# typesense/typesense

Hardware: AMD Instinct MI355X
Metric: queries/sec, 10M-doc keyword 3-term AND top-100 (Topster 250) (higher is better)
Workload: dtype u32/i64

## Files before the change

### typesense_amd/csrc/kw_find2.hip.h

```cpp
#pragma once

#ifndef TSGPU_F2_SPAN
#define TSGPU_F2_SPAN 12
#endif
#ifndef TSGPU_F2_FAST
#define TSGPU_F2_FAST 1
#endif
static const int KW_F2_SPAN = TSGPU_F2_SPAN;
#ifndef TSGPU_F2_WAVES
#define TSGPU_F2_WAVES 7
#endif
#ifdef TSGPU_HIP_EMU
#define KW_F2_WAVES
#else
#define KW_F2_WAVES __attribute__((amdgpu_waves_per_eu(TSGPU_F2_WAVES)))
#endif
#ifndef TSGPU_F2_QUAD
#define TSGPU_F2_QUAD 0
#endif
static const bool KW_F2_QUAD = TSGPU_F2_QUAD != 0;
static const bool KW_F2_FAST = TSGPU_F2_FAST != 0;
#ifndef TSGPU_F2_MIDSLABS
#define TSGPU_F2_MIDSLABS 0
#endif
// ... 6 lines not shown
#else
#define KW_F2_LOOP_BARRIER() __syncthreads()
#endif


template <int TMAX, bool COUNT = false>
__device__ __forceinline__ void kw_find2_body(const IndexView& ix, const KwQueryDev* __restrict__ queries, const KwWorkItem* __restrict__ work, const KwPartials& part,
                                              uint32_t* __restrict__ hits_all, const uint64_t* __restrict__ hit_off, const uint32_t bid) {
    __shared__ KwSmem<TMAX, 512, false, true, true> sm;
    __shared__ uint32_t wave_cnt_b[2][KW_THREADS / 64];
    uint32_t* __restrict__ hits = hits_all + hit_off[bid] * (uint64_t)(TMAX + 1);
    __shared__ KwQueryDev sq;
    const uint32_t t = threadIdx.x;
    const KwWorkItem wi = work[bid];
    uint32_t cb_ids = 0, cb_meta = 0, cb_tile = 0, cb_probe = 0, cb_rec = 0;
    {
        const uint32_t* src = (const uint32_t*)(queries + wi.query);
        uint32_t* dst = (uint32_t*)&sq;
        for (uint32_t i = t; i < sizeof(KwQueryDev) / 4; i += KW_THREADS) { dst[i] = src[i]; if constexpr (COUNT) cb_meta += 4; }
    }
    if (t == 0) { sm.q1_cnt = 0; sm.qf_cnt = 0; sm.tk_cnt = 0; sm.have_thr = 0; sm.n_match = 0; sm.n_emit = 0; sm.off_words = 0; }
    __syncthreads();
    const KwQueryDev& q = sq;
    const uint32_t T = q.n_lists;
    const ListDesc dA = ix.lists[q.list[q.probe_order[0]]];
    const ListDesc dB = ix.lists[q.list[q.probe_order[T >= 2 ? 1 : 0]]];
    const uint32_t* __restrict__ blB = ix.blk_last + dB.blk_base;
    const BlockIds* __restrict__ biA = ix.blk_ids + dA.blk_base;
    const BlockIds* __restrict__ biB = ix.blk_ids + dB.blk_base;
    const uint32_t* __restrict__ idwA = ix.ids_payload + dA.ids_base;
    const uint32_t* __restrict__ idwB = ix.ids_payload + dB.ids_base;
    const uint32_t lane = t & 63, wave = t >> 6;
    const BlockIds PAD = {0xFFFFFFFFu, 0xFFFFFFFFu, 0u, 0u};
    if constexpr (COUNT) { if (lane == 0) cb_meta += 2 * (uint32_t)sizeof(ListDesc) + 16; }

    auto load_id_raw = [&](const BlockIds& m, uint32_t slot) -> uint32_t {
        const uint32_t n = m.n_ids_bits & 0xFFFF;
        const uint32_t s2 = slot < n ? slot : 0;
        const uint32_t* __restrict__ w = idwA + m.ids_woff;
        if constexpr (COUNT) { if (slot < n) cb_ids += (m.n_ids_bits >> 16) == 16 ? 2u : 4u; }
        return (m.n_ids_bits >> 16) == 16 ? (uint32_t)((const uint16_t*)w)[s2] : w[s2];
    };
    const uint32_t nB = T >= 2 ? dB.n_blocks : 0u;
    auto load_window = [&](uint32_t base) -> BlockIds {
        if constexpr (COUNT) { if (base + lane < nB) cb_meta += 16; }
        return base + lane < nB ? biB[base + lane] : PAD;
    };
    uint32_t abase = wi.blk_begin;
    auto load_awin = [&](uint32_t base) -> BlockIds { const uint32_t bb = base + lane; if constexpr (COUNT) { if (bb < wi.blk_end) cb_meta += 16; } return biA[bb < wi.blk_end ? bb : wi.blk_end - 1]; };
    BlockIds awin = load_awin(abase);
    auto meta = [&](uint32_t bb) -> BlockIds {
        const int j = (int)((bb < wi.blk_end ? bb : wi.blk_end - 1) - abase);
        BlockIds m;
        m.first_id = (uint32_t)__builtin_amdgcn_readlane((int)awin.first_id, j);
        m.last_id = (uint32_t)__builtin_amdgcn_readlane((int)awin.last_id, j);
        m.ids_woff = (uint32_t)__builtin_amdgcn_readlane((int)awin.ids_woff, j);
        m.n_ids_bits = (uint32_t)__builtin_amdgcn_readlane((int)awin.n_ids_bits, j);
        return m;
    };

    uint32_t wbase = 0, wver = 0;
    BlockIds win = load_window(0), nxt = load_window(32);
    uint32_t win_dirty = 1;
    struct Plan { uint32_t mode, rlo, rhi, w_begin, W, ver, base, buf; };
    constexpr int PIPE_WORDS = KW_FIND_PIPE_WORDS;
    constexpr int TILE_WORDS = KW_FIND_TILE_WORDS;
    static_assert(TILE_WORDS == 2 * PIPE_WORDS * KW_THREADS, "two tile buffers: one searched, one being filled");
    constexpr int HALF = PIPE_WORDS * KW_THREADS;
    uint32_t tbuf = 0;
    auto make_plan = [&](uint32_t lo_id, uint32_t hi_id) -> Plan {
        Plan P; P.mode = 4; P.rlo = P.rhi = P.w_begin = P.W = 0; P.ver = wver; P.base = wbase; P.buf = 0;
        if (T < 2) return P;
        unsigned long long mk = __ballot(win.last_id >= lo_id ? 1 : 0);
        if (mk != 0 && (uint32_t)__builtin_ctzll(mk) >= 32) {
            wbase += 32; win = nxt; nxt = load_window(wbase + 32); win_dirty = 1;
            mk = __ballot(win.last_id >= lo_id ? 1 : 0);
        }
        if (mk == 0) {
            uint32_t lo = wbase + 64, hi = dB.n_blocks;
            while (lo < hi) { const uint32_t mid = (lo + hi) >> 1; if constexpr (COUNT) { if (lane == 0) cb_meta += 4; } if (blB[mid] >= lo_id) hi = mid; else lo = mid + 1; }
            wbase = lo; win = load_window(wbase); nxt = load_window(wbase + 32); win_dirty = 1;
            mk = __ballot(win.last_id >= lo_id ? 1 : 0);
        }
        P.rlo = (uint32_t)__builtin_ctzll(mk);
        P.base = wbase;
        if (wbase + P.rlo >= dB.n_blocks) { P.mode = 3; return P; }
        const unsigned long long mh = __ballot(win.last_id >= hi_id ? 1 : 0);
// ... 5 lines not shown
            if (t < 64) { sm.bw_last[wver][t] = win.last_id; sm.bw_first[wver][t] = win.first_id; sm.bw_woff[wver][t] = win.ids_woff; sm.bw_nb[wver][t] = win.n_ids_bits; }
            win_dirty = 0;
        }
        P.ver = wver;
        uint32_t has_breaks = dB.flags & LIST_HAS_BREAKS;
        KW_UNIFORM_OPAQUE(has_breaks);
        if (has_breaks) {
            const uint32_t w_endw = win.ids_woff + packed_words(win.n_ids_bits & 0xFFFF, win.n_ids_bits >> 16);
            const uint32_t nxt_woff = (uint32_t)__shfl(win.ids_woff, (int)((lane + 1) & 63));
            const bool brk = lane >= P.rlo && lane < P.rhi && w_endw != nxt_woff;
            if (__ballot(brk ? 1 : 0) != 0) { P.mode = 2; return P; }
        }
        P.w_begin = (uint32_t)__builtin_amdgcn_readlane((int)win.ids_woff, (int)P.rlo);
        const uint32_t nb_hi = (uint32_t)__builtin_amdgcn_readlane((int)win.n_ids_bits, (int)P.rhi);
        P.W = (uint32_t)__builtin_amdgcn_readlane((int)win.ids_woff, (int)P.rhi) + packed_words(nb_hi & 0xFFFF, nb_hi >> 16) - P.w_begin;
        if (P.W <= (uint32_t)(PIPE_WORDS * KW_THREADS)) {
            P.mode = 0;
            tbuf ^= 1; P.buf = tbuf;
            const uint32_t* lane_src = idwB + P.w_begin + t;
            uint32_t* lds_wave_base = sm.btile + tbuf * HALF + wave * 64;
#if TSGPU_F2_MIDSLABS
            if (P.W <= 2u * KW_THREADS) kw_glds_slabs<2>(lane_src, lds_wave_base);
            else if (PIPE_WORDS > 4 && P.W <= 4u * KW_THREADS) kw_glds_slabs<4>(lane_src, lds_wave_base);
            else kw_glds_slabs<PIPE_WORDS>(lane_src, lds_wave_base);
            if constexpr (COUNT) cb_tile += 4u * (P.W <= 2u * KW_THREADS ? 2u : ((PIPE_WORDS > 4 && P.W <= 4u * KW_THREADS) ? 4u : (uint32_t)PIPE_WORDS));
#else
            if (P.W <= 2u * KW_THREADS) kw_glds_slabs<2>(lane_src, lds_wave_base);
            else kw_glds_slabs<PIPE_WORDS>(lane_src, lds_wave_base);
            if constexpr (COUNT) cb_tile += 4u * (P.W <= 2u * KW_THREADS ? 2u : (uint32_t)PIPE_WORDS);
#endif
        } else P.mode = KW_F2_ROUNDS ? 1 : 2;
        return P;
    };

    uint32_t a_first, a_nb, b_first, b_nb;
    uint32_t araw0, araw1;
    Plan P;
    {
        const BlockIds mA = meta(wi.blk_begin), mB = meta(wi.blk_begin + 1);
        araw0 = load_id_raw(mA, t); araw1 = load_id_raw(mB, t);
        P = make_plan(mA.first_id, wi.blk_begin + 1 < wi.blk_end ? mB.last_id : mA.last_id);
        a_first = mA.first_id; a_nb = mA.n_ids_bits; b_first = mB.first_id; b_nb = mB.n_ids_bits;
    }
    const uint32_t has_deadline = q.deadline_rem_us;
    uint32_t q1n = 0, qfn = 0, par = 0, qh = 0;
    KW_PROF_DECL
// ... 33 lines not shown
    auto drain_q1 = [&]() { while (q1n >= (uint32_t)KW_THREADS) probe_batch(KW_THREADS); };

    for (uint32_t b = wi.blk_begin, it = 0; b < wi.blk_end; b += 2, it++) {
        if (P.mode == 3) break;
        uint32_t Tl = T;
        KW_UNIFORM_OPAQUE(Tl);
        KW_PROF(8)
        kw_glds_wait();
        KW_PROF(1)
        if (has_deadline) { if ((it & 7) == 0 && kw_out_of_time<true>(KW_RELOAD_VIEW(ix), q, wi.query, &sm.stop)) break; }
        const bool two = b + 1 < wi.blk_end;
        const uint32_t n0 = a_nb & 0xFFFF, n1 = two ? (b_nb & 0xFFFF) : 0u;
        bool ok0 = t < n0, ok1 = t < n1;
        const uint32_t id0 = ok0 ? a_first + araw0 : 0xFFFFFFFFu, id1 = ok1 ? b_first + araw1 : 0xFFFFFFFFu;
        const Plan C = P;
        KW_PROF(0)
        const uint32_t* __restrict__ tile = sm.btile + C.buf * HALF;
        KW_F2_LOOP_BARRIER();
        KW_PROF(2)
        const uint32_t cur_last = win.last_id;
        uint32_t araw0n = 0, araw1n = 0;
        if (b + 2 < wi.blk_end) {
            const BlockIds mC = meta(b + 2), mD = meta(b + 3);
            araw0n = load_id_raw(mC, t);
            araw1n = load_id_raw(mD, t);
            KW_PROF(10)
            P = make_plan(mC.first_id, b + 3 < wi.blk_end ? mD.last_id : mC.last_id);
            a_first = mC.first_id; a_nb = mC.n_ids_bits; b_first = mD.first_id; b_nb = mD.n_ids_bits;
        }
        KW_PROF(4)
// ... 109 lines not shown
                while (r_hi < C.rhi && woff[r_hi + 1] + packed_words(wnb[r_hi + 1] & 0xFFFF, wnb[r_hi + 1] >> 16) - w_begin <= (uint32_t)HALF) r_hi++;
                const uint32_t W = woff[r_hi] + packed_words(wnb[r_hi] & 0xFFFF, wnb[r_hi] >> 16) - w_begin;
                const uint32_t* __restrict__ src = idwB + w_begin;
                __syncthreads();
                for (uint32_t i0 = t; i0 < W + t; i0 += 2 * KW_THREADS) {
                    const uint32_t i1 = i0 + KW_THREADS;
                    const uint32_t c0 = src[i0 < W ? i0 : 0], c1 = src[i1 < W ? i1 : 0];
                    if (i0 < W) rt[i0] = c0;
                    if (i1 < W) rt[i1] = c1;
                }
                __syncthreads();
                if (!done0 && pos0 >= r_lo && pos0 <= r_hi) { slot_search(rt, id0, first0, nb0, woff[pos0] - w_begin, pos0, found0, p10); done0 = true; }
                if (!done1 && pos1 >= r_lo && pos1 <= r_hi) { slot_search(rt, id1, first1, nb1, woff[pos1] - w_begin, pos1, found1, p11); done1 = true; }
                r_lo = r_hi + 1;
            }
        } else if (C.mode == 2) {
            const IndexView ixp = KW_RELOAD_VIEW(ix);
            const ListDesc dBp = ixp.lists[q.list[q.probe_order[1]]];
            if constexpr (COUNT) {
                if (ok0) found0 = probe_list<true>(ixp, dBp, id0, p10, &cb_probe);
                if (ok1) found1 = probe_list<true>(ixp, dBp, id1, p11, &cb_probe);
            } else {
                ProbeReq r0, r1;
                r0.e = make_uint2(0u, 0u); r0.state = 0; r1.e = make_uint2(0u, 0u); r1.state = 0;
                if (ok0) probe_issue(ixp, dBp, id0, r0);
                if (ok1) probe_issue(ixp, dBp, id1, r1);
                if (ok0) found0 = probe_finish(ixp, dBp, id0, r0, p10);
                if (ok1) found1 = probe_finish(ixp, dBp, id1, r1, p11);
            }
        }
// ... 46 lines not shown
        }
        KW_PROF(7)
        if (b + 5 >= abase + 64 && b + 4 < wi.blk_end) { abase = b + 4; awin = load_awin(abase); }
        araw0 = araw0n; araw1 = araw1n;
    }
    if (T >= 3) while (q1n > 0) probe_batch(q1n < (uint32_t)KW_THREADS ? q1n : (uint32_t)KW_THREADS);
    if (t == 0) part.cnt[bid] = qfn;
    if constexpr (COUNT) {
        uint32_t c[5] = {cb_ids, cb_meta, cb_tile, cb_probe, cb_rec};
#pragma unroll
        for (int k = 0; k < 5; k++) {
            for (int m = 32; m > 0; m >>= 1) c[k] += __shfl_xor(c[k], m);
            if (lane == 0 && ix.touched) atomicAdd(ix.touched + k, (unsigned long long)c[k]);
        }
        if (t == 0 && ix.touched) { atomicAdd(ix.touched + 5, 1ull); atomicAdd(ix.touched + 6, (unsigned long long)qfn); }
    }
    KW_PROF(9)
    KW_PROF_FLUSH(ix.prof)
}

template <int TMAX, bool COUNT = false>
__global__ __launch_bounds__(KW_THREADS) KW_F2_WAVES void kw_find2_kernel(IndexView ix, const KwQueryDev* __restrict__ queries,
                                                                                      const KwWorkItem* __restrict__ work, KwPartials part,
                                                                                      uint32_t* __restrict__ hits_all, const uint64_t* __restrict__ hit_off) {
    kw_find2_body<TMAX, COUNT>(ix, queries, work, part, hits_all, hit_off, blockIdx.x);
}
```

### typesense_amd/csrc/kw_kernels.hip.h

```cpp
#pragma once
#include <hip/hip_runtime.h>
#include <stdint.h>
#include "tsgpu_format.h"

#include <type_traits>

namespace tsgpu {

#ifdef TSGPU_PROF
#define KW_PROF_DECL unsigned long long prof_t[12] = {0,0,0,0,0,0,0,0,0,0,0,0}; unsigned long long prof_last = __builtin_readcyclecounter();
#define KW_PROF(i) { const unsigned long long _n = __builtin_readcyclecounter(); prof_t[i] += _n - prof_last; prof_last = _n; }
#define KW_PROF_FLUSH(ptr) if (threadIdx.x == 0 && (ptr)) { for (int _i = 0; _i < 12; _i++) atomicAdd((ptr) + _i, prof_t[_i]); atomicAdd((ptr) + 12, 1ull); }
#else
#define KW_PROF_DECL
#define KW_PROF(i)
#define KW_PROF_FLUSH(ptr)
#endif

#ifndef TSGPU_SCORE_WAVES
#define TSGPU_SCORE_WAVES 6
#endif
#ifndef TSGPU_SCORE_MF_WAVES
#define TSGPU_SCORE_MF_WAVES 4
#endif
// ... 61 lines not shown
    const uint32_t* ids_payload;
    const uint32_t* payload;
    const int64_t* const* columns;
    const uint32_t* column_len;
    uint32_t n_columns;
    uint32_t num_docs;
    const uint2* iddir;
    uint32_t iddir_slot_entries;
    uint32_t iddir_cap_ids;
    unsigned long long* prof;
    unsigned long long* touched;
    const struct KwQueryMF* mf;
    uint32_t* fbits;
    const long long* t0;
    uint32_t ticks_per_us;
    uint32_t* cutoff;
    const SortKeyDesc* sort_keys;
};

#if defined(TSGPU_HIP_EMU) || defined(TSGPU_NO_KERNARG_RELOAD)
#define KW_RELOAD_VIEW(ix) (ix)
#else
__device__ __forceinline__ IndexView kw_reload_view_from_kernarg(const IndexView& ix) {
#if defined(__HIP_DEVICE_COMPILE__)
    typedef const __attribute__((address_space(4))) uint32_t* KernargWords;
    KernargWords p = (KernargWords)__builtin_amdgcn_kernarg_segment_ptr();
    asm volatile("" : "+s"(p));
    union { IndexView v; uint32_t w[sizeof(IndexView) / 4]; } u;
    static_assert(sizeof(IndexView) % 4 == 0, "copied as dwords");
#pragma unroll
// ... 2937 lines not shown
```

### typesense_amd/csrc/tsgpu.hip

```cpp
#include "tsgpu_host.h"
#if defined(__linux__)
#include <sys/prctl.h>
#include <time.h>
#endif
#include <cmath>
#include "kw_kernels.hip.h"
#include "kw_plan.hip.h"

using namespace tsgpu;

namespace {


uint64_t now_us() {
    return (uint64_t)std::chrono::duration_cast<std::chrono::microseconds>(
               std::chrono::system_clock::now().time_since_epoch()).count();
}

int upload(DevBuf& dst, const void* src, size_t bytes, hipStream_t s) {
    int rc = dst.reserve(bytes ? bytes : 16);
    if (rc) return rc;
    if (bytes) TSGPU_HIP_TRY(hipMemcpyAsync(dst.p, src, bytes, hipMemcpyHostToDevice, s));
    return TSGPU_OK;
}
// ... 27 lines not shown
    v.blk_meta = sn.ar ? sn.ar->blk_meta.as<BlockMeta>() : nullptr;
    v.ids_payload = sn.ar ? sn.ar->ids_payload.as<uint32_t>() : nullptr;
    v.payload = sn.ar ? sn.ar->payload.as<uint32_t>() : nullptr;
    v.columns = ctx->d_col_ptrs.as<const int64_t*>();
    v.column_len = ctx->d_col_len.as<uint32_t>();
    v.n_columns = (uint32_t)ctx->columns.size();
    v.num_docs = ctx->num_docs;
    v.iddir = sn.dir_pool ? sn.dir_pool->buf.as<uint2>() : nullptr;
    v.iddir_slot_entries = sn.dir_pool ? sn.dir_pool->slot_entries : 0u;
    v.iddir_cap_ids = sn.dir_pool ? sn.dir_pool->cap_ids : 0u;
    v.prof = ctx->d_prof.as<unsigned long long>();
    v.touched = nullptr;
    v.mf = nullptr;
    v.fbits = nullptr;
    v.t0 = nullptr; v.ticks_per_us = 100; v.cutoff = nullptr;
    v.sort_keys = ctx->d_sort_keys.as<SortKeyDesc>();
    return v;
}

template <int TMAX, int CAP>
void launch_search(hipStream_t s, uint32_t n_work, const IndexView& v, const KwQueryDev* q, const KwWorkItem* w,
                   const KwPartials& part, const uint32_t* aux, uint32_t* ids_out, bool s2) {
    if (CAP == 512 && !s2) hipLaunchKernelGGL((kw_search_kernel<TMAX, CAP, CAP != 512>), dim3(n_work), dim3(KW_THREADS), 0, s, v, q, w, part, aux, ids_out, (uint32_t*)nullptr, (const uint64_t*)nullptr);
    else hipLaunchKernelGGL((kw_search_kernel<TMAX, CAP, true>), dim3(n_work), dim3(KW_THREADS), 0, s, v, q, w, part, aux, ids_out, (uint32_t*)nullptr, (const uint64_t*)nullptr);
}

template <int TMAX>
void launch_find_score(int cap, hipStream_t s, uint32_t n_work, const IndexView& v, const KwQueryDev* q, const KwWorkItem* w, const KwPartials& part,
                       const uint32_t* aux, uint32_t* ids_out, bool s2, uint32_t* hits, const uint64_t* hit_off, hipEvent_t mid_ev = nullptr, bool pair = false, bool plain = false) {
    if (pair && v.touched) hipLaunchKernelGGL((kw_find2_kernel<TMAX, true>), dim3(n_work), dim3(KW_THREADS), 0, s, v, q, w, part, hits, hit_off);
// ... 260 lines not shown
    if (!strcmp(name, "kw_cost_fixed")) { ctx->kw_cost_fixed = (uint32_t)std::max<int64_t>(value, 0); return ok(); }
    if (!strcmp(name, "kw_sort_work")) { ctx->kw_sort_work = value != 0; return ok(); }
    if (!strcmp(name, "kw_two_kernels")) { ctx->kw_two_kernels = value != 0; return ok(); }
    if (!strcmp(name, "sortkey_dense_div")) {
        if (value < 0 || value > (1ll << 31)) return fail(TSGPU_ERR_INVALID, "sortkey_dense_div out of range (0..2^31)");
        std::lock_guard<std::mutex> sk(ctx->sk_mu);
        ctx->sortkey_dense_div = value; return ok();
    }
    if (!strcmp(name, "kw_device_plan_min_queries")) { ctx->kw_device_plan_min_queries = (uint32_t)std::min<int64_t>(std::max<int64_t>(value, 0), 1 << 30); return ok(); }
    if (!strcmp(name, "kw_pair_blocks")) { ctx->kw_pair_blocks = value != 0; return ok(); }
    if (!strcmp(name, "doc_range_lo")) { ctx->doc_range_set = true; ctx->doc_range_lo = (uint32_t)std::min<int64_t>(std::max<int64_t>(value, 0), 0xFFFFFFFFll); return ok(); }
    if (!strcmp(name, "doc_range_hi")) { ctx->doc_range_set = true; ctx->doc_range_hi = (uint32_t)std::min<int64_t>(std::max<int64_t>(value, 0), 0xFFFFFFFFll); return ok(); }
    if (!strcmp(name, "kw_candidates_rank_fold")) { ctx->kw_candidates_rank_fold = value != 0; return ok(); }
    if (!strcmp(name, "kw_mf_pipelined")) { ctx->kw_mf_pipelined = value != 0; return ok(); }
    if (!strcmp(name, "kw_count_touched")) { ctx->kw_count_touched = value != 0; return ok(); }
    if (!strcmp(name, "kw_iddir_min_ids")) { ctx->kw_iddir_min_ids = value < 0 ? 0 : value; ctx->commit_force_full = true; return ok(); }
    if (!strcmp(name, "kw_iddir_density_div")) { ctx->kw_iddir_density_div = value < 1 ? 1 : value; ctx->commit_force_full = true; return ok(); }
    if (!strcmp(name, "kw_iddir_budget_mb")) { ctx->kw_iddir_budget_mb = value < 0 ? 0 : value; ctx->commit_force_full = true; return ok(); }
    if (!strcmp(name, "kw_host_split_tail_slices")) { ctx->kw_host_split_tail_slices = value >= 2 ? 2 : 1; return ok(); }
    if (!strcmp(name, "kw_host_split_device_plan")) { ctx->kw_host_split_device_plan = value != 0; return ok(); }
    if (!strcmp(name, "kw_host_split_first_pct")) { ctx->kw_host_split_first_pct = (uint32_t)std::min<int64_t>(95, std::max<int64_t>(5, value)); return ok(); }
    if (!strcmp(name, "kw_host_split_queries")) { ctx->kw_host_split_queries = (uint32_t)std::max<int64_t>(0, value); return ok(); }
    if (!strcmp(name, "kw_zero_copy_max_queries")) { ctx->kw_zero_copy_max_queries = (uint32_t)std::max<int64_t>(0, value); return ok(); }
    if (!strcmp(name, "kw_timing_min_queries")) { ctx->kw_timing_min_queries = (uint32_t)std::max<int64_t>(0, value); return ok(); }
    if (!strcmp(name, "kw_merge_select_min")) { ctx->kw_merge_select_min = (uint32_t)std::max<int64_t>(0, value); return ok(); }
    if (!strcmp(name, "hnsw_visited_hash")) { ctx->hnsw_visited_hash = value != 0; return ok(); }
    if (!strcmp(name, "hnsw_test_tiny_cand")) { ctx->hnsw_test_tiny_cand = value != 0; return ok(); }
    if (!strcmp(name, "hnsw_visited_max_gib")) { ctx->hnsw_visited_max_gib = (int)std::min<int64_t>(std::max<int64_t>(1, value), 128); return ok(); }
    if (!strcmp(name, "blocking_sync_min_callers")) { ctx->blocking_sync_min_callers = (int)std::max<int64_t>(0, value); return ok(); }
    if (!strcmp(name, "plan_threads")) { if (value < 1 || value > 64) return fail(TSGPU_ERR_INVALID, "plan_threads: 1..64"); ctx->plan_threads = (int)value; return ok(); }
// ... 85 lines not shown
    if (!strcmp(name, "kw_max_plan_us")) { *out = ctx->kw_max_plan_us.exchange(0); return ok(); }
    if (!strcmp(name, "kw_max_upload_us")) { *out = ctx->kw_max_upload_us.exchange(0); return ok(); }
    if (!strcmp(name, "kw_max_launch_us")) { *out = ctx->kw_max_launch_us.exchange(0); return ok(); }
    if (!strcmp(name, "kw_max_wait_us")) { *out = ctx->kw_max_wait_us.exchange(0); return ok(); }
    if (!strcmp(name, "kw_queue_us")) { *out = ctx->kw_queue_us.load(); return ok(); }
    if (!strcmp(name, "kw_wake_us")) { *out = ctx->kw_wake_us.load(); return ok(); }
    if (!strcmp(name, "kw_max_queue_us")) { *out = ctx->kw_max_queue_us.exchange(0); return ok(); }
    if (!strcmp(name, "kw_max_wake_us")) { *out = ctx->kw_max_wake_us.exchange(0); return ok(); }
    if (!strcmp(name, "kw_upload_us")) { *out = ctx->kw_upload_us.load(); return ok(); }
    if (!strcmp(name, "kw_launch_us")) { *out = ctx->kw_launch_us.load(); return ok(); }
    if (!strcmp(name, "kw_wait_us")) { *out = ctx->kw_wait_us.load(); return ok(); }
    if (!strcmp(name, "kw_book_us")) { *out = ctx->kw_book_us.load(); return ok(); }
    if (!strcmp(name, "kw_device_plans")) { *out = ctx->kw_device_plans.load(); return ok(); }
    if (!strcmp(name, "kw_device_plan_fallbacks")) { *out = ctx->kw_device_plan_fallbacks.load(); return ok(); }
    if (!strcmp(name, "sort_keys_live")) { *out = ctx->sort_keys_live.load(); return ok(); }
    if (!strcmp(name, "kw_iddir_built")) { *out = ctx->kw_iddir_built; return ok(); }
    if (!strcmp(name, "kw_iddir_lists")) { const auto sn = ctx->snapshot(); uint64_t n = 0; if (sn) for (const auto& r : sn->dir_of) n += r ? 1 : 0; *out = n; return ok(); }
    if (!strcmp(name, "batch_exec_us")) { *out = ctx->batch_exec_us.load(); return ok(); }
    if (!strcmp(name, "batch_scatter_us")) { *out = ctx->batch_scatter_us.load(); return ok(); }
    if (!strcmp(name, "batch_rounds")) { *out = ctx->kw_comb.rounds + ctx->vec_comb.rounds; return ok(); }
    if (!strcmp(name, "gb_batch_rounds")) { *out = ctx->gb_comb.rounds; return ok(); }
    if (!strcmp(name, "gb_batch_coalesced_calls")) { *out = ctx->gb_comb.coalesced_calls; return ok(); }
    if (!strcmp(name, "batch_coalesced_calls")) { *out = ctx->kw_comb.coalesced_calls + ctx->vec_comb.coalesced_calls; return ok(); }
    return fail(TSGPU_ERR_NOT_FOUND, std::string("tsgpu_get_counter: unknown counter ") + name);
}

int tsgpu_keep_result_ids(tsgpu_ctx* ctx, int keep) {
    if (!ctx) return fail(TSGPU_ERR_INVALID, "ctx is NULL");
    std::lock_guard<std::mutex> lk(ctx->mu);
    ctx->keep_ids = keep != 0;
// ... 903 lines not shown
    v.mf = T.mf;
    if (P.fbits_words) {
        if ((rc = L.d_fbits.reserve(P.fbits_words * 4))) return rc;
        TSGPU_HIP_TRY(hipMemsetAsync(L.d_fbits.p, 0, P.fbits_words * 4, s));
    }
    v.fbits = L.d_fbits.as<uint32_t>();
    if ((rc = L.d_t0.reserve(64))) return rc;
    v.t0 = L.d_t0.as<long long>(); v.ticks_per_us = ctx->ticks_per_us;
    if (P.any_deadline) {
        if ((rc = L.d_cut.reserve((size_t)n_queries * 4))) return rc;
        TSGPU_HIP_TRY(hipMemsetAsync(L.d_cut.p, 0, (size_t)n_queries * 4, s));
        hipLaunchKernelGGL(kw_stamp_kernel, dim3(1), dim3(1), 0, s, L.d_t0.as<long long>());
    }
    v.cutoff = L.d_cut.as<uint32_t>();
    if (count_touched) {
        if ((rc = L.d_touched.reserve(8 * 8))) return rc;
        TSGPU_HIP_TRY(hipMemsetAsync(L.d_touched.p, 0, 8 * 8, s));
        v.touched = L.d_touched.as<unsigned long long>();
    }
    const KwQueryDev* dq = T.dq; const KwWorkItem* dw = T.dw; const uint32_t* daux = T.daux; uint32_t* ids_out = T.ids_out;
    if (timing) TSGPU_HIP_TRY(hipEventRecord(L.ev[0], s));
    auto run_table = [&](int tb, auto tmax_tag, auto mf_tag) {
        constexpr int TM = decltype(tmax_tag)::value;
        constexpr bool MFT = decltype(mf_tag)::value;
        const size_t nws = H.n[tb], first = H.first[tb];
        const TablePlan& tp = H.tp[tb];
        if (nws == 0) return;
        if (tp.two) {
            st.hit_groups += (uint32_t)tp.group_start.size() - 1;
            for (size_t gi = 0; gi + 1 < tp.group_start.size(); gi++) {
                const size_t a = tp.group_start[gi], b = tp.group_start[gi + 1];
                if (b <= a) continue;
// ... 85 lines not shown

void record_timings(tsgpu_ctx* ctx, KwLane& L, bool timing, const LaunchStats& st, uint64_t hit_records, const Plan& P, bool dev_plan, const tsgpu_kw_query* queries,
                    const std::vector<uint64_t>& off_words, const uint64_t* num_matched) {
    float ms_a = 0, ms_b = 0, ms_find = 0;
    if (timing) { (void)hipEventElapsedTime(&ms_a, L.ev[0], L.ev[1]); (void)hipEventElapsedTime(&ms_b, L.ev[1], L.ev[2]); }
    if (timing && st.find_marked && st.hit_groups == 1) (void)hipEventElapsedTime(&ms_find, L.ev[0], L.ev[3]);
    uint64_t bytes = P.list_bytes;
    for (uint32_t i = 0; i < off_words.size(); i++) bytes += 4ull * off_words[i] + (num_matched ? 8ull * num_matched[i] * n_column_sort_keys(P, dev_plan, queries, i) : 0);
    std::lock_guard<std::mutex> tl(ctx->tm_mu);
    ctx->timings.kw_search_ms = ms_a; ctx->timings.kw_merge_ms = ms_b; ctx->timings.kw_find_ms = ms_find; ctx->timings.total_ms = ms_a + ms_b;
    ctx->timings.kw_algorithmic_bytes = bytes;
    ctx->kw_last_hit_groups = st.hit_groups; ctx->kw_last_hit_records = hit_records;
}

int record_touched(tsgpu_ctx* ctx, KwLane& L, const Plan& P, bool dev_plan, const tsgpu_kw_query* queries, uint32_t n_queries, const uint64_t* nm, const uint64_t* nm_dev) {
    uint64_t c[8];
    TSGPU_HIP_TRY(hipMemcpy(c, L.d_touched.p, sizeof(c), hipMemcpyDeviceToHost));
    std::lock_guard<std::mutex> tl(ctx->tm_mu);
    tsgpu_kw_touched& tt = ctx->kw_touched;
    tt.find_driver_ids = c[0]; tt.find_metadata = c[1]; tt.find_tile_dma = c[2]; tt.find_probes = c[3]; tt.find_records = c[4];
    tt.find_work_items = c[5]; tt.find_hit_records = c[6];
    tt.find_requested_bytes = c[0] + c[1] + c[2] + c[3] + c[4];
    uint64_t sb = 0;
    std::vector<uint64_t> nm_host;
    if (nm_dev) {
        nm_host.resize(n_queries);
        if (hipMemcpy(nm_host.data(), nm_dev, (size_t)n_queries * 8, hipMemcpyDeviceToHost) == hipSuccess) nm = nm_host.data();
    }
    for (uint32_t i = 0; nm && !dev_plan && i < n_queries; i++)
        sb += nm[i] * (4ull * ((P.q[i].n_lists <= 3 ? 3 : KW_MAX_TOKENS) + 1) + 56ull * P.q[i].n_lists + 8ull * n_column_sort_keys(P, dev_plan, queries, i));
    tt.score_requested_bytes = sb;
    return TSGPU_OK;
}
// ... 656 lines not shown
```

### typesense_amd/csrc/tsgpu_format.h

```cpp
#pragma once
#include <stdint.h>

#if defined(__HIPCC__) || defined(TSGPU_HIP_EMU)
#define TSGPU_HD __host__ __device__
#else
#define TSGPU_HD
#endif

namespace tsgpu {

static const uint32_t BLOCK_IDS = 256;

struct BlockIds {
    uint32_t first_id;
    uint32_t last_id;
    uint32_t ids_woff;
    uint32_t n_ids_bits;
};

struct BlockMeta {
    uint32_t first_id;
    uint32_t ids_woff;
    uint32_t oi_woff;
    uint32_t off_woff;
// ... 11 lines not shown
struct ListDesc {
    uint64_t payload_base;
    uint64_t ids_base;
    uint32_t blk_base;
    uint32_t n_blocks;
    uint32_t n_ids;
    uint32_t first_id;
    uint32_t last_id;
    uint32_t n_off;
    uint32_t flags;
    uint32_t dir_slot;
};
static const uint32_t LIST_HAS_BREAKS = 1u;

static const uint32_t IDDIR_SPLIT = 0x80000000u;

TSGPU_HD static inline uint32_t required_bits(uint32_t v) {
    return v == 0 ? 0u : 32u - (uint32_t)__builtin_clz(v);
}

TSGPU_HD static inline uint32_t packed_words(uint32_t n, uint32_t bits) {
    return (uint32_t)(((uint64_t)n * bits + 31) / 32) + 1;
}

TSGPU_HD static inline uint32_t unpack_at(const uint32_t* __restrict__ w, uint32_t idx, uint32_t bits) {
    if (bits == 0) return 0;
    const uint64_t bitpos = (uint64_t)idx * bits;
    const uint64_t wi = bitpos >> 5;
    const uint32_t sh = (uint32_t)(bitpos & 31);
    const uint64_t two = (uint64_t)w[wi] | ((uint64_t)w[wi + 1] << 32);
// ... 6 lines not shown
```

### typesense_amd/csrc/tsgpu_host.h

```cpp
#pragma once
#include <hip/hip_runtime.h>
#include <cstdint>
#include <cstdio>
#include <cstring>
#include <string>
#include <deque>
#include <functional>
#include <vector>
#include <mutex>
#include <condition_variable>
#include <memory>
#include <atomic>
#include <thread>
#include <utility>
#include <unordered_map>
#include <algorithm>
#include <chrono>
#include <new>
#include <exception>
#include "../../include/tsgpu.h"
#include "tsgpu_format.h"
#include "tsgpu_pack.h"
#include "tsgpu_batcher.h"

// ... 450 lines not shown
    tsgpu::DevBuf d_prof;
    bool keep_ids = false;
    uint32_t kw_max_partials = 16;
    uint32_t kw_cost_r_x10 = 10, kw_cost_probe_x100 = 20;
    uint32_t kw_cost_fixed = 16;
    bool kw_sort_work = true;
    uint32_t kw_host_split_queries = 1000;
    bool kw_host_split_device_plan = true;
    uint32_t kw_host_split_tail_slices = 1;
    uint32_t kw_host_split_first_pct = 85;
    uint32_t kw_zero_copy_max_queries = 256;
    uint32_t kw_timing_min_queries = 64;
    uint32_t kw_merge_select_min = 2;
    bool kw_count_touched = false;
    tsgpu_kw_touched kw_touched{};
    std::atomic<uint64_t> kw_mf_pipelined_launches{0}, kw_candidates_rank_launches{0};
    bool kw_candidates_rank_fold = true;
    bool kw_mf_pipelined = true;
    bool kw_pair_blocks = true;
    bool doc_range_set = false; uint32_t doc_range_lo = 0, doc_range_hi = 0;
    long long kw_iddir_min_ids = 256;
    long long kw_iddir_density_div = 64;
    long long kw_iddir_budget_mb = 4096;
    uint64_t kw_iddir_built = 0;
    bool kw_two_kernels = true;
    uint32_t kw_device_plan_min_queries = 512;
    std::atomic<uint64_t> kw_device_plans{0}, kw_device_plan_fallbacks{0};
    uint32_t kw_hit_buffer_mb = 20480;
    uint32_t kw_last_hit_groups = 0;
    uint64_t kw_hit_buffer_records = 0, kw_last_hit_records = 0;
    uint32_t kw_chunk_blocks = 0;
    uint32_t vec_rows_per_slab = 0;
    uint32_t vec_sample_tiles = 0;
    uint32_t vec_cand_cap = 0;
    uint64_t commit_failed_count = 0;
    uint32_t vec_ip_lanes = 4;
    uint32_t vec_prefilter = 1;
    uint64_t vec_prefilter_groups = 0;
    int hnsw_test_tiny_cand = 0;
// ... 94 lines not shown
```

### typesense_amd/csrc/tsgpu_index.hip

```cpp
#include "tsgpu_host.h"

using namespace tsgpu;

namespace {

uint64_t wall_us() { return (uint64_t)std::chrono::duration_cast<std::chrono::microseconds>(std::chrono::steady_clock::now().time_since_epoch()).count(); }

const char* validate_list(const uint32_t* ids, const uint64_t* oi, uint32_t n_ids, uint64_t n_off) {
    if (n_ids == 0) return nullptr;
    if (oi[n_ids - 1] >= n_off) return "offset_index beyond offsets (every document needs at least one offset)";
    for (uint32_t i = 1; i < n_ids; i++) {
        if (ids[i] <= ids[i - 1]) return "ids must be strictly ascending";
        if (oi[i] <= oi[i - 1]) return "offset_index must be strictly ascending (every document needs at least one offset)";
    }
    return nullptr;
}

inline uint32_t ids_words(const BlockMeta& m) { return packed_words(m.n_ids, m.ids_bits); }
inline uint32_t pay_words(const BlockMeta& m) { return packed_words(m.n_ids, m.oi_bits) + packed_words(m.n_off, m.off_bits); }

void mark_dirty(tsgpu_ctx* ctx, uint32_t field, uint32_t term, TermHost* t) {
    ctx->dirty = true;
    if (t && t->queued) return;
    if (t) { t->dirty = true; t->queued = true; }
// ... 287 lines not shown
    t.garbage_idw = t.pl.ids_payload.size() + 4096;
    t.garbage_pw = t.pl.payload.size() + 4096;
}

__global__ void index_desc_scatter_kernel(const uint64_t* __restrict__ dst, const uint32_t* __restrict__ last, const BlockIds* __restrict__ bids,
                                          const BlockMeta* __restrict__ bmeta, uint32_t n, uint32_t* a_last, BlockIds* a_bids, BlockMeta* a_bmeta) {
    const uint32_t i = blockIdx.x * blockDim.x + threadIdx.x;
    if (i >= n) return;
    const uint64_t d = dst[i];
    a_last[d] = last[i]; a_bids[d] = bids[i]; a_bmeta[d] = bmeta[i];
}

struct IdDirJob { uint64_t ids_base; uint64_t first_block; uint32_t blk_base, n_blocks, slot, pad; };

__global__ __launch_bounds__(256) void index_iddir_build_kernel(const IdDirJob* __restrict__ jobs, uint32_t n_jobs, const BlockIds* __restrict__ blk_ids,
                                                                const uint32_t* __restrict__ ids_payload, uint2* __restrict__ dir, uint32_t slot_entries, uint32_t cap_ids) {
    const uint64_t gb = blockIdx.x;
    uint32_t lo = 0, hi = n_jobs - 1;
    while (lo < hi) { const uint32_t mid = (lo + hi + 1) >> 1; if (jobs[mid].first_block <= gb) lo = mid; else hi = mid - 1; }
    const IdDirJob j = jobs[lo];
    const uint32_t b = (uint32_t)(gb - j.first_block);
    const BlockIds m = blk_ids[j.blk_base + b];
    const uint32_t n = m.n_ids_bits & 0xFFFF, t = threadIdx.x;
    if (t >= n) return;
    const uint32_t* __restrict__ w = ids_payload + j.ids_base + m.ids_woff;
    const bool w16 = (m.n_ids_bits >> 16) == 16;
    const uint32_t id = m.first_id + (w16 ? (uint32_t)((const uint16_t*)w)[t] : w[t]);
    if (id >= cap_ids) return;
    unsigned int* e = (unsigned int*)(dir + (size_t)j.slot * slot_entries + (id >> 5));
    bool lowest;
    if (t == 0) {
        const bool shared = b > 0 && (blk_ids[j.blk_base + b - 1].last_id >> 5) == (id >> 5);
        if (shared) atomicOr(e, IDDIR_SPLIT);
        lowest = !shared;
    } else lowest = ((m.first_id + (w16 ? (uint32_t)((const uint16_t*)w)[t - 1] : w[t - 1])) >> 5) != (id >> 5);
    if (lowest) atomicOr(e, b * (uint32_t)BLOCK_IDS + t);
    atomicOr(e + 1, 1u << (id & 31u));
}

int build_id_directories(tsgpu_ctx* ctx, Snapshot& s, const Snapshot* cur, const std::vector<uint32_t>* touched, uint32_t num_docs) {
    for (ListDesc& d : s.h_lists) d.dir_slot = 0;
    s.dir_pool.reset(); s.dir_of.clear();
    if (ctx->kw_iddir_min_ids <= 0 || ctx->kw_iddir_budget_mb <= 0 || !s.ar || s.h_lists.empty()) return TSGPU_OK;
    uint64_t id_lo = ~0ull, id_hi = 0;
    for (const ListDesc& d : s.h_lists) if (d.n_ids) { id_lo = std::min<uint64_t>(id_lo, d.first_id); id_hi = std::max<uint64_t>(id_hi, d.last_id); }
    const uint64_t id_span = id_hi >= id_lo ? std::min<uint64_t>(id_hi - id_lo + 1, num_docs ? num_docs : ~0ull) : num_docs;
    const uint64_t thr = std::max<uint64_t>((uint64_t)ctx->kw_iddir_min_ids, id_span / (uint64_t)ctx->kw_iddir_density_div);
    std::vector<uint32_t> want;
    for (size_t h = 0; h < s.h_lists.size(); h++) if (s.h_lists[h].n_ids >= thr && s.h_lists[h].n_blocks) want.push_back((uint32_t)h);
    if (want.empty()) return TSGPU_OK;
    std::sort(want.begin(), want.end(), [&](uint32_t a, uint32_t b) { return s.h_lists[a].n_ids != s.h_lists[b].n_ids ? s.h_lists[a].n_ids > s.h_lists[b].n_ids : a < b; });
    std::shared_ptr<IdDirPool> pool = (cur && touched && cur->dir_pool && num_docs <= cur->dir_pool->cap_ids) ? cur->dir_pool : nullptr;
    const bool reuse = (bool)pool;
    if (!pool) {
        const uint64_t cap = ((uint64_t)num_docs + num_docs / 8 + 1024 + 2047) / 2048 * 2048;
        if (cap > 0xFFFFF000ull) return TSGPU_OK;
        const uint64_t slot_bytes = cap / 32 * sizeof(uint2);
        const uint64_t n_slots = std::min<uint64_t>((uint64_t)ctx->kw_iddir_budget_mb * (1ull << 20) / slot_bytes, 2 * want.size() + 8);
        if (n_slots == 0) return TSGPU_OK;
        pool = std::make_shared<IdDirPool>();
        pool->bin = ctx->retire_bin;
        if (pool->buf.reserve(n_slots * slot_bytes) != TSGPU_OK) { tls_error().clear(); return TSGPU_OK; }
        pool->cap_ids = (uint32_t)cap; pool->slot_entries = (uint32_t)(cap / 32); pool->n_slots = (uint32_t)n_slots;
        for (uint32_t i = (uint32_t)n_slots; i-- > 0;) pool->free_slots.push_back(i);
    }
    if (want.size() > (size_t)pool->n_slots / 2 + 4) want.resize((size_t)pool->n_slots / 2 + 4);
    std::vector<uint8_t> is_touched;
    if (touched) { is_touched.assign(s.h_lists.size(), 0); for (uint32_t h : *touched) if (h < is_touched.size()) is_touched[h] = 1; }
    s.dir_of.assign(s.h_lists.size(), nullptr);
    std::vector<IdDirJob> jobs;
    uint64_t total_blocks = 0;
    for (uint32_t h : want) {
        if (reuse && h < cur->dir_of.size() && cur->dir_of[h] && !is_touched[h]) { s.dir_of[h] = cur->dir_of[h]; continue; }
        uint32_t slot;
        if (!pool->take(slot)) continue;
        s.dir_of[h] = std::make_shared<IdDirRef>(pool, slot);
        const ListDesc& d = s.h_lists[h];
        jobs.push_back({d.ids_base, total_blocks, d.blk_base, d.n_blocks, slot, 0u});
        total_blocks += d.n_blocks;
    }
    if (!jobs.empty()) {
        if (total_blocks > 0x7FFFFFFFull) { s.dir_of.clear(); return TSGPU_OK; }
        DevBuf d_jobs;
        int rc = d_jobs.reserve(jobs.size() * sizeof(IdDirJob));
        if (rc != TSGPU_OK) { s.dir_of.clear(); tls_error().clear(); return TSGPU_OK; }
        hipError_t e = hipMemcpy(d_jobs.p, jobs.data(), jobs.size() * sizeof(IdDirJob), hipMemcpyHostToDevice);
        for (size_t i = 0; i < jobs.size() && e == hipSuccess; i++)
            e = hipMemsetAsync(pool->buf.as<uint2>() + (size_t)jobs[i].slot * pool->slot_entries, 0, (size_t)pool->slot_entries * sizeof(uint2), ctx->stream);
        if (e == hipSuccess) {
            hipLaunchKernelGGL(index_iddir_build_kernel, dim3((uint32_t)total_blocks), dim3(256), 0, ctx->stream, d_jobs.as<IdDirJob>(), (uint32_t)jobs.size(), s.ar->blk_ids.as<BlockIds>(),
                               s.ar->ids_payload.as<uint32_t>(), pool->buf.as<uint2>(), pool->slot_entries, pool->cap_ids);
            e = hipGetLastError();
            if (e == hipSuccess) e = hipStreamSynchronize(ctx->stream);
        }
        d_jobs.release();
        if (e != hipSuccess) { s.dir_of.clear(); return fail(TSGPU_ERR_DEVICE, std::string("tsgpu_commit: id directories: ") + hipGetErrorString(e)); }
        ctx->kw_iddir_built += jobs.size();
    }
    s.dir_pool = pool;
    for (size_t h = 0; h < s.dir_of.size(); h++) if (s.dir_of[h]) s.h_lists[h].dir_slot = s.dir_of[h]->slot + 1;
    return TSGPU_OK;
}

int commit_full(tsgpu_ctx* ctx) {
    std::shared_ptr<Snapshot> sp = std::make_shared<Snapshot>();
    sp->bin = ctx->retire_bin;
    Snapshot& s = *sp;
    std::shared_ptr<ArenaSet> ar = std::make_shared<ArenaSet>();
    ar->bin = ctx->retire_bin;
    std::shared_ptr<HandleMaps> maps = std::make_shared<HandleMaps>();
    std::vector<std::pair<uint64_t, TermHost*>> order;
    for (auto& f : ctx->fields) {
// ... 340 lines not shown
```

Baseline: 1.354 million.

## Probe second list through id-directory bitmap tiles in find kernel

When the second list has a bitmap id directory and the work item's id span is dense enough, the find kernel streams directory entries (offset plus 32-bit bitmap) into the LDS tile. Each id is then resolved with a bit test and popcount instead of walking block windows and searching slots. Split entries fall back to the normal probe path. The directory build now marks an entry as split only when the preceding block is partial, which should reduce fallbacks. The directory buffer gets over-read padding, and the change adds counters and tunable knobs.

```diff
diff --git a/typesense_amd/csrc/kw_find2.hip.h b/typesense_amd/csrc/kw_find2.hip.h
--- a/typesense_amd/csrc/kw_find2.hip.h
+++ b/typesense_amd/csrc/kw_find2.hip.h
@@ -44,6 +44,7 @@
     const uint32_t t = threadIdx.x;
     const KwWorkItem wi = work[bid];
     uint32_t cb_ids = 0, cb_meta = 0, cb_tile = 0, cb_probe = 0, cb_rec = 0;
+    uint32_t cn_pairs = 0, cn_dir = 0, cn_wide = 0;
     {
         const uint32_t* src = (const uint32_t*)(queries + wi.query);
         uint32_t* dst = (uint32_t*)&sq;
@@ -71,11 +72,6 @@
         if constexpr (COUNT) { if (slot < n) cb_ids += (m.n_ids_bits >> 16) == 16 ? 2u : 4u; }
         return (m.n_ids_bits >> 16) == 16 ? (uint32_t)((const uint16_t*)w)[s2] : w[s2];
     };
-    const uint32_t nB = T >= 2 ? dB.n_blocks : 0u;
-    auto load_window = [&](uint32_t base) -> BlockIds {
-        if constexpr (COUNT) { if (base + lane < nB) cb_meta += 16; }
-        return base + lane < nB ? biB[base + lane] : PAD;
-    };
     uint32_t abase = wi.blk_begin;
     auto load_awin = [&](uint32_t base) -> BlockIds { const uint32_t bb = base + lane; if constexpr (COUNT) { if (bb < wi.blk_end) cb_meta += 16; } return biA[bb < wi.blk_end ? bb : wi.blk_end - 1]; };
     BlockIds awin = load_awin(abase);
@@ -89,6 +85,24 @@
         return m;
     };
 
+    uint32_t dmode = 0;
+    const uint32_t* __restrict__ tsrc = idwB;
+    if (T >= 2 && dB.dir_slot != 0 && ix.find_dir_span != 0) {
+        const uint32_t item_first = (uint32_t)__builtin_amdgcn_readlane((int)awin.first_id, 0), item_last = biA[wi.blk_end - 1].last_id;
+        const uint32_t pairs = (wi.blk_end - wi.blk_begin + 1) >> 1;
+        if constexpr (COUNT) { if (lane == 0) cb_meta += 16; }
+        if (item_last < ix.iddir_cap_ids && (unsigned long long)(item_last - item_first) <= (unsigned long long)ix.find_dir_span * pairs) {
+            dmode = 1;
+            tsrc = (const uint32_t*)(ix.iddir + (size_t)(dB.dir_slot - 1) * ix.iddir_slot_entries);
+        }
+    }
+    KW_UNIFORM_OPAQUE(dmode);
+    const uint32_t nB = (T >= 2 && !dmode) ? dB.n_blocks : 0u;
+    auto load_window = [&](uint32_t base) -> BlockIds {
+        if constexpr (COUNT) { if (base + lane < nB) cb_meta += 16; }
+        return base + lane < nB ? biB[base + lane] : PAD;
+    };
+
     uint32_t wbase = 0, wver = 0;
     BlockIds win = load_window(0), nxt = load_window(32);
     uint32_t win_dirty = 1;
@@ -96,11 +110,18 @@
     constexpr int PIPE_WORDS = KW_FIND_PIPE_WORDS;
     constexpr int TILE_WORDS = KW_FIND_TILE_WORDS;
     static_assert(TILE_WORDS == 2 * PIPE_WORDS * KW_THREADS, "two tile buffers: one searched, one being filled");
+    static_assert(PIPE_WORDS * KW_THREADS * 4 <= (int)KW_DIR_TILE_OVERREAD_BYTES, "a directory-tile fill reads at most this far past its slice");
     constexpr int HALF = PIPE_WORDS * KW_THREADS;
     uint32_t tbuf = 0;
     auto make_plan = [&](uint32_t lo_id, uint32_t hi_id) -> Plan {
         Plan P; P.mode = 4; P.rlo = P.rhi = P.w_begin = P.W = 0; P.ver = wver; P.base = wbase; P.buf = 0;
         if (T < 2) return P;
+        if (dmode) {
+            P.rlo = lo_id >> 5;
+            P.w_begin = 2u * P.rlo;
+            P.W = 2u * ((hi_id >> 5) - P.rlo + 1u);
+            P.mode = 2;
+        } else {
         unsigned long long mk = __ballot(win.last_id >= lo_id ? 1 : 0);
         if (mk != 0 && (uint32_t)__builtin_ctzll(mk) >= 32) {
             wbase += 32; win = nxt; nxt = load_window(wbase + 32); win_dirty = 1;
@@ -136,10 +157,12 @@
         P.w_begin = (uint32_t)__builtin_amdgcn_readlane((int)win.ids_woff, (int)P.rlo);
         const uint32_t nb_hi = (uint32_t)__builtin_amdgcn_readlane((int)win.n_ids_bits, (int)P.rhi);
         P.W = (uint32_t)__builtin_amdgcn_readlane((int)win.ids_woff, (int)P.rhi) + packed_words(nb_hi & 0xFFFF, nb_hi >> 16) - P.w_begin;
+        P.mode = KW_F2_ROUNDS ? 1 : 2;
+        }
         if (P.W <= (uint32_t)(PIPE_WORDS * KW_THREADS)) {
-            P.mode = 0;
+            P.mode = dmode ? 5 : 0;
             tbuf ^= 1; P.buf = tbuf;
-            const uint32_t* lane_src = idwB + P.w_begin + t;
+            const uint32_t* lane_src = tsrc + P.w_begin + t;
             uint32_t* lds_wave_base = sm.btile + tbuf * HALF + wave * 64;
 #if TSGPU_F2_MIDSLABS
             if (P.W <= 2u * KW_THREADS) kw_glds_slabs<2>(lane_src, lds_wave_base);
@@ -151,7 +174,7 @@
             else kw_glds_slabs<PIPE_WORDS>(lane_src, lds_wave_base);
             if constexpr (COUNT) cb_tile += 4u * (P.W <= 2u * KW_THREADS ? 2u : (uint32_t)PIPE_WORDS);
 #endif
-        } else P.mode = KW_F2_ROUNDS ? 1 : 2;
+        }
         return P;
     };
 
@@ -215,6 +238,7 @@
         bool ok0 = t < n0, ok1 = t < n1;
         const uint32_t id0 = ok0 ? a_first + araw0 : 0xFFFFFFFFu, id1 = ok1 ? b_first + araw1 : 0xFFFFFFFFu;
         const Plan C = P;
+        if constexpr (COUNT) { cn_pairs++; cn_dir += C.mode == 5 ? 1u : 0u; cn_wide += (dmode && C.mode == 2) ? 1u : 0u; }
         KW_PROF(0)
         const uint32_t* __restrict__ tile = sm.btile + C.buf * HALF;
         KW_F2_LOOP_BARRIER();
@@ -354,6 +378,25 @@
                 if (!done1 && pos1 >= r_lo && pos1 <= r_hi) { slot_search(rt, id1, first1, nb1, woff[pos1] - w_begin, pos1, found1, p11); done1 = true; }
                 r_lo = r_hi + 1;
             }
+        } else if (C.mode == 5) {
+            const uint32_t k0 = ok0 ? 2u * ((id0 >> 5) - C.rlo) : 0u, k1 = ok1 ? 2u * ((id1 >> 5) - C.rlo) : 0u;
+            const uint2 e0 = make_uint2(tile[k0], tile[k0 + 1]), e1 = make_uint2(tile[k1], tile[k1 + 1]);
+            const uint32_t bit0 = 1u << (id0 & 31u), bit1 = 1u << (id1 & 31u);
+            const bool in0 = ok0 && (e0.y & bit0) != 0, in1 = ok1 && (e1.y & bit1) != 0;
+            const bool slow0 = in0 && (e0.x & IDDIR_SPLIT) != 0, slow1 = in1 && (e1.x & IDDIR_SPLIT) != 0;
+            p10 = e0.x + (uint32_t)__popc(e0.y & (bit0 - 1u)); p11 = e1.x + (uint32_t)__popc(e1.y & (bit1 - 1u));
+            found0 = in0 && !slow0; found1 = in1 && !slow1;
+            if (__ballot((slow0 || slow1) ? 1 : 0) != 0) {
+                const IndexView ixp = KW_RELOAD_VIEW(ix);
+                const ListDesc dBp = ixp.lists[q.list[q.probe_order[1]]];
+                if constexpr (COUNT) {
+                    if (slow0) found0 = probe_list<true>(ixp, dBp, id0, p10, &cb_probe);
+                    if (slow1) found1 = probe_list<true>(ixp, dBp, id1, p11, &cb_probe);
+                } else {
+                    if (slow0) found0 = probe_search(ixp, dBp, id0, p10);
+                    if (slow1) found1 = probe_search(ixp, dBp, id1, p11);
+                }
+            }
         } else if (C.mode == 2) {
             const IndexView ixp = KW_RELOAD_VIEW(ix);
             const ListDesc dBp = ixp.lists[q.list[q.probe_order[1]]];
@@ -430,6 +473,10 @@
             if (lane == 0 && ix.touched) atomicAdd(ix.touched + k, (unsigned long long)c[k]);
         }
         if (t == 0 && ix.touched) { atomicAdd(ix.touched + 5, 1ull); atomicAdd(ix.touched + 6, (unsigned long long)qfn); }
+        if (t == 0 && ix.touched) {
+            atomicAdd(ix.touched + 7, (unsigned long long)dmode); atomicAdd(ix.touched + 8, (unsigned long long)cn_pairs);
+            atomicAdd(ix.touched + 9, (unsigned long long)cn_dir); atomicAdd(ix.touched + 10, (unsigned long long)cn_wide);
+        }
     }
     KW_PROF(9)
     KW_PROF_FLUSH(ix.prof)
diff --git a/typesense_amd/csrc/kw_kernels.hip.h b/typesense_amd/csrc/kw_kernels.hip.h
--- a/typesense_amd/csrc/kw_kernels.hip.h
+++ b/typesense_amd/csrc/kw_kernels.hip.h
@@ -99,6 +99,7 @@
     uint32_t* fbits;
     const long long* t0;
     uint32_t ticks_per_us;
+    uint32_t find_dir_span;
     uint32_t* cutoff;
     const SortKeyDesc* sort_keys;
 };
diff --git a/typesense_amd/csrc/tsgpu.hip b/typesense_amd/csrc/tsgpu.hip
--- a/typesense_amd/csrc/tsgpu.hip
+++ b/typesense_amd/csrc/tsgpu.hip
@@ -65,6 +65,7 @@
     v.mf = nullptr;
     v.fbits = nullptr;
     v.t0 = nullptr; v.ticks_per_us = 100; v.cutoff = nullptr;
+    v.find_dir_span = ctx->kw_find_dir_tile ? (uint32_t)(ctx->kw_find_dir_span_pct * (long long)(KW_FIND_PIPE_WORDS * KW_THREADS * 16) / 100) : 0u;
     v.sort_keys = ctx->d_sort_keys.as<SortKeyDesc>();
     return v;
 }
@@ -355,6 +356,8 @@
     if (!strcmp(name, "kw_candidates_rank_fold")) { ctx->kw_candidates_rank_fold = value != 0; return ok(); }
     if (!strcmp(name, "kw_mf_pipelined")) { ctx->kw_mf_pipelined = value != 0; return ok(); }
     if (!strcmp(name, "kw_count_touched")) { ctx->kw_count_touched = value != 0; return ok(); }
+    if (!strcmp(name, "kw_find_dir_tile")) { ctx->kw_find_dir_tile = value != 0; return ok(); }
+    if (!strcmp(name, "kw_find_dir_span_pct")) { ctx->kw_find_dir_span_pct = std::min<int64_t>(std::max<int64_t>(value, 1), 1 << 20); return ok(); }
     if (!strcmp(name, "kw_iddir_min_ids")) { ctx->kw_iddir_min_ids = value < 0 ? 0 : value; ctx->commit_force_full = true; return ok(); }
     if (!strcmp(name, "kw_iddir_density_div")) { ctx->kw_iddir_density_div = value < 1 ? 1 : value; ctx->commit_force_full = true; return ok(); }
     if (!strcmp(name, "kw_iddir_budget_mb")) { ctx->kw_iddir_budget_mb = value < 0 ? 0 : value; ctx->commit_force_full = true; return ok(); }
@@ -470,6 +473,11 @@
     if (!strcmp(name, "kw_device_plans")) { *out = ctx->kw_device_plans.load(); return ok(); }
     if (!strcmp(name, "kw_device_plan_fallbacks")) { *out = ctx->kw_device_plan_fallbacks.load(); return ok(); }
     if (!strcmp(name, "sort_keys_live")) { *out = ctx->sort_keys_live.load(); return ok(); }
+    if (!strcmp(name, "kw_find_dir_items")) { *out = ctx->kw_find_dir_items; return ok(); }
+    if (!strcmp(name, "kw_find_pairs")) { *out = ctx->kw_find_pairs; return ok(); }
+    if (!strcmp(name, "kw_find_dir_pairs")) { *out = ctx->kw_find_dir_pairs; return ok(); }
+    if (!strcmp(name, "kw_find_dir_wide_pairs")) { *out = ctx->kw_find_dir_wide_pairs; return ok(); }
+    if (!strcmp(name, "kw_iddir_split_entries")) { *out = ctx->kw_iddir_split_entries; return ok(); }
     if (!strcmp(name, "kw_iddir_built")) { *out = ctx->kw_iddir_built; return ok(); }
     if (!strcmp(name, "kw_iddir_lists")) { const auto sn = ctx->snapshot(); uint64_t n = 0; if (sn) for (const auto& r : sn->dir_of) n += r ? 1 : 0; *out = n; return ok(); }
     if (!strcmp(name, "batch_exec_us")) { *out = ctx->batch_exec_us.load(); return ok(); }
@@ -1403,8 +1411,8 @@
     }
     v.cutoff = L.d_cut.as<uint32_t>();
     if (count_touched) {
-        if ((rc = L.d_touched.reserve(8 * 8))) return rc;
-        TSGPU_HIP_TRY(hipMemsetAsync(L.d_touched.p, 0, 8 * 8, s));
+        if ((rc = L.d_touched.reserve(12 * 8))) return rc;
+        TSGPU_HIP_TRY(hipMemsetAsync(L.d_touched.p, 0, 12 * 8, s));
         v.touched = L.d_touched.as<unsigned long long>();
     }
     const KwQueryDev* dq = T.dq; const KwWorkItem* dw = T.dw; const uint32_t* daux = T.daux; uint32_t* ids_out = T.ids_out;
@@ -1520,9 +1528,10 @@
 }
 
 int record_touched(tsgpu_ctx* ctx, KwLane& L, const Plan& P, bool dev_plan, const tsgpu_kw_query* queries, uint32_t n_queries, const uint64_t* nm, const uint64_t* nm_dev) {
-    uint64_t c[8];
+    uint64_t c[12];
     TSGPU_HIP_TRY(hipMemcpy(c, L.d_touched.p, sizeof(c), hipMemcpyDeviceToHost));
     std::lock_guard<std::mutex> tl(ctx->tm_mu);
+    ctx->kw_find_dir_items = c[7]; ctx->kw_find_pairs = c[8]; ctx->kw_find_dir_pairs = c[9]; ctx->kw_find_dir_wide_pairs = c[10];
     tsgpu_kw_touched& tt = ctx->kw_touched;
     tt.find_driver_ids = c[0]; tt.find_metadata = c[1]; tt.find_tile_dma = c[2]; tt.find_probes = c[3]; tt.find_records = c[4];
     tt.find_work_items = c[5]; tt.find_hit_records = c[6];
diff --git a/typesense_amd/csrc/tsgpu_format.h b/typesense_amd/csrc/tsgpu_format.h
--- a/typesense_amd/csrc/tsgpu_format.h
+++ b/typesense_amd/csrc/tsgpu_format.h
@@ -49,6 +49,7 @@
 static const uint32_t LIST_HAS_BREAKS = 1u;
 
 static const uint32_t IDDIR_SPLIT = 0x80000000u;
+static const uint32_t KW_DIR_TILE_OVERREAD_BYTES = 8192;
 
 TSGPU_HD static inline uint32_t required_bits(uint32_t v) {
     return v == 0 ? 0u : 32u - (uint32_t)__builtin_clz(v);
diff --git a/typesense_amd/csrc/tsgpu_host.h b/typesense_amd/csrc/tsgpu_host.h
--- a/typesense_amd/csrc/tsgpu_host.h
+++ b/typesense_amd/csrc/tsgpu_host.h
@@ -488,6 +488,7 @@
     uint32_t kw_merge_select_min = 2;
     bool kw_count_touched = false;
     tsgpu_kw_touched kw_touched{};
+    uint64_t kw_find_dir_items = 0, kw_find_pairs = 0, kw_find_dir_pairs = 0, kw_find_dir_wide_pairs = 0;
     std::atomic<uint64_t> kw_mf_pipelined_launches{0}, kw_candidates_rank_launches{0};
     bool kw_candidates_rank_fold = true;
     bool kw_mf_pipelined = true;
@@ -497,6 +498,9 @@
     long long kw_iddir_density_div = 64;
     long long kw_iddir_budget_mb = 4096;
     uint64_t kw_iddir_built = 0;
+    uint64_t kw_iddir_split_entries = 0;
+    bool kw_find_dir_tile = true;
+    long long kw_find_dir_span_pct = 80;
     bool kw_two_kernels = true;
     uint32_t kw_device_plan_min_queries = 512;
     std::atomic<uint64_t> kw_device_plans{0}, kw_device_plan_fallbacks{0};
diff --git a/typesense_amd/csrc/tsgpu_index.hip b/typesense_amd/csrc/tsgpu_index.hip
--- a/typesense_amd/csrc/tsgpu_index.hip
+++ b/typesense_amd/csrc/tsgpu_index.hip
@@ -325,7 +325,8 @@
 struct IdDirJob { uint64_t ids_base; uint64_t first_block; uint32_t blk_base, n_blocks, slot, pad; };
 
 __global__ __launch_bounds__(256) void index_iddir_build_kernel(const IdDirJob* __restrict__ jobs, uint32_t n_jobs, const BlockIds* __restrict__ blk_ids,
-                                                                const uint32_t* __restrict__ ids_payload, uint2* __restrict__ dir, uint32_t slot_entries, uint32_t cap_ids) {
+                                                                const uint32_t* __restrict__ ids_payload, uint2* __restrict__ dir, uint32_t slot_entries, uint32_t cap_ids,
+                                                                unsigned long long* __restrict__ split_entries) {
     const uint64_t gb = blockIdx.x;
     uint32_t lo = 0, hi = n_jobs - 1;
     while (lo < hi) { const uint32_t mid = (lo + hi + 1) >> 1; if (jobs[mid].first_block <= gb) lo = mid; else hi = mid - 1; }
@@ -341,8 +342,9 @@
     unsigned int* e = (unsigned int*)(dir + (size_t)j.slot * slot_entries + (id >> 5));
     bool lowest;
     if (t == 0) {
-        const bool shared = b > 0 && (blk_ids[j.blk_base + b - 1].last_id >> 5) == (id >> 5);
-        if (shared) atomicOr(e, IDDIR_SPLIT);
+        bool shared = false, part = false;
+        if (b > 0) { const BlockIds pm = blk_ids[j.blk_base + b - 1]; shared = (pm.last_id >> 5) == (id >> 5); part = (pm.n_ids_bits & 0xFFFF) < BLOCK_IDS; }
+        if (shared && part && !(atomicOr(e, IDDIR_SPLIT) & IDDIR_SPLIT)) atomicAdd(split_entries, 1ull);
         lowest = !shared;
     } else lowest = ((m.first_id + (w16 ? (uint32_t)((const uint16_t*)w)[t - 1] : w[t - 1])) >> 5) != (id >> 5);
     if (lowest) atomicOr(e, b * (uint32_t)BLOCK_IDS + t);
@@ -371,7 +373,7 @@
         if (n_slots == 0) return TSGPU_OK;
         pool = std::make_shared<IdDirPool>();
         pool->bin = ctx->retire_bin;
-        if (pool->buf.reserve(n_slots * slot_bytes) != TSGPU_OK) { tls_error().clear(); return TSGPU_OK; }
+        if (pool->buf.reserve(n_slots * slot_bytes + KW_DIR_TILE_OVERREAD_BYTES) != TSGPU_OK) { tls_error().clear(); return TSGPU_OK; }
         pool->cap_ids = (uint32_t)cap; pool->slot_entries = (uint32_t)(cap / 32); pool->n_slots = (uint32_t)n_slots;
         for (uint32_t i = (uint32_t)n_slots; i-- > 0;) pool->free_slots.push_back(i);
     }
@@ -393,20 +395,25 @@
     if (!jobs.empty()) {
         if (total_blocks > 0x7FFFFFFFull) { s.dir_of.clear(); return TSGPU_OK; }
         DevBuf d_jobs;
-        int rc = d_jobs.reserve(jobs.size() * sizeof(IdDirJob));
+        int rc = d_jobs.reserve((jobs.size() + 1) * sizeof(IdDirJob));
         if (rc != TSGPU_OK) { s.dir_of.clear(); tls_error().clear(); return TSGPU_OK; }
+        unsigned long long* d_splits = (unsigned long long*)(d_jobs.as<IdDirJob>() + jobs.size());
+        unsigned long long n_splits = 0;
         hipError_t e = hipMemcpy(d_jobs.p, jobs.data(), jobs.size() * sizeof(IdDirJob), hipMemcpyHostToDevice);
+        if (e == hipSuccess) e = hipMemsetAsync(d_splits, 0, sizeof(unsigned long long), ctx->stream);
         for (size_t i = 0; i < jobs.size() && e == hipSuccess; i++)
             e = hipMemsetAsync(pool->buf.as<uint2>() + (size_t)jobs[i].slot * pool->slot_entries, 0, (size_t)pool->slot_entries * sizeof(uint2), ctx->stream);
         if (e == hipSuccess) {
             hipLaunchKernelGGL(index_iddir_build_kernel, dim3((uint32_t)total_blocks), dim3(256), 0, ctx->stream, d_jobs.as<IdDirJob>(), (uint32_t)jobs.size(), s.ar->blk_ids.as<BlockIds>(),
-                               s.ar->ids_payload.as<uint32_t>(), pool->buf.as<uint2>(), pool->slot_entries, pool->cap_ids);
+                               s.ar->ids_payload.as<uint32_t>(), pool->buf.as<uint2>(), pool->slot_entries, pool->cap_ids, d_splits);
             e = hipGetLastError();
             if (e == hipSuccess) e = hipStreamSynchronize(ctx->stream);
+            if (e == hipSuccess) e = hipMemcpy(&n_splits, d_splits, sizeof(n_splits), hipMemcpyDeviceToHost);
         }
         d_jobs.release();
         if (e != hipSuccess) { s.dir_of.clear(); return fail(TSGPU_ERR_DEVICE, std::string("tsgpu_commit: id directories: ") + hipGetErrorString(e)); }
         ctx->kw_iddir_built += jobs.size();
+        ctx->kw_iddir_split_entries += n_splits;
     }
     s.dir_pool = pool;
     for (size_t h = 0; h < s.dir_of.size(); h++) if (s.dir_of[h]) s.h_lists[h].dir_slot = s.dir_of[h]->slot + 1;
```

Measured after the change: 1.556 million, median of 6. +14.9%, better.
